# vvvm23/distributed-pytorch-cookbook

Measured on AMD Instinct MI355X. Metric: tokens/sec (node) GPT-2 training per recipe (DDP/FSDP/PP) at 1/2/4/8 MI355X, higher is better.
Workload: dtype bf16; 1 GPU; model=gpt2-small, global_batch=64, seq_len=1024, parallelism=dp1, recipe=main-ddp.py, reduce_dtype=fp32, pp_comm_dtype=fp32, step_graph=True

## Files before the change

### distributed_pytorch_cookbook_amd/ops/csrc/attention.hip

```cpp
#include "common.h"

#include <cstdlib>
#include <type_traits>

namespace dpc {

struct AttnArgs {
  const void* q; const void* k; const void* v;
  void* o;
  float* lse;
  const unsigned char* pad;
  const void* dout;
  void* dq; void* dk; void* dv;
  float* delta;
  long long ld_qkv, ld_o, ld_dqkv;
  int N, S, H;
  float scale;
  int causal;
  int hd;
  int order;
};

constexpr int KT = 64;
constexpr int QB = 128;
// ... 65 lines not shown
__device__ __forceinline__ void dma_voff(int (&v)[AT<HD>::NPW], long long ld, int wid, int lane) {
#pragma unroll
  for (int i = 0; i < AT<HD>::NPW; ++i) {
    const int prow = 8 * (wid * AT<HD>::NPW + i) + (lane >> 3);
    const int e = prow * 64 + (((lane & 7) ^ aswz(prow)) << 3);
    const int row = e / HD, chunk = (e % HD) >> 3;
    v[i] = (int)((long long)row * ld * 2 + chunk * 16);
  }
}

template <int HD>
__device__ __forceinline__ void tile_dma(const bf16_t* base, long long ld, int row0, int S, bool valid,
                                         const int (&v)[AT<HD>::NPW], bf16_t* lds, int wid) {
  const __amdgpu_buffer_rsrc_t rs = rows_rsrc(base, (unsigned)(ld * 2), row0, S, valid);
#pragma unroll
  for (int i = 0; i < AT<HD>::NPW; ++i) dma16(rs, v[i], lds + (wid * AT<HD>::NPW + i) * 512);
}

template <int HD>
__device__ __forceinline__ bf16x8 row_frag(const bf16_t* lds, int row0, int st, int lane) {
  return *reinterpret_cast<const bf16x8*>(lds + toff<HD>(row0 + (lane & 31), 2 * st + (lane >> 5)));
}

template <int HD>
__device__ __forceinline__ bf16x8 tr_frag(const bf16_t* lds, int r0, int s, int c0, int lane) {
  const int h = lane >> 5, g2 = (lane >> 4) & 1, i16 = lane & 15, q = i16 >> 2, p = i16 & 3;
  const int row = r0 + 16 * s + 4 * h + q;
  const int col = c0 + 16 * g2 + 4 * p;
  const bf16_t* a0 = lds + toff<HD>(row, col >> 3) + (col & 7);
  const bf16_t* a1 = lds + toff<HD>(row + 8, col >> 3) + (col & 7);
  short4_t lo = __builtin_amdgcn_ds_read_tr16_b64_v4i16((lds4_t)a0);
  short4_t hi = __builtin_amdgcn_ds_read_tr16_b64_v4i16((lds4_t)a1);
  typedef short short8_t __attribute__((ext_vector_type(8)));
  short8_t s8 = {lo[0], lo[1], lo[2], lo[3], hi[0], hi[1], hi[2], hi[3]};
  return __builtin_bit_cast(bf16x8, s8);
}

__device__ __forceinline__ bf16x8 acc_frag(const floatx16& x, int s) {
  uint4 u;
  u.x = pack2bf(x[8 * s + 0], x[8 * s + 1]);
  u.y = pack2bf(x[8 * s + 2], x[8 * s + 3]);
  u.z = pack2bf(x[8 * s + 4], x[8 * s + 5]);
  u.w = pack2bf(x[8 * s + 6], x[8 * s + 7]);
  return __builtin_bit_cast(bf16x8, u);
}

__device__ __forceinline__ int acc_row(int r, int lane) { return (r & 3) + 8 * (r >> 2) + 4 * (lane >> 5); }

__device__ __forceinline__ void store_pair16(bf16_t* row, int g, int hh, uint2 wa, uint2 wb) {
  const auto s0 = __builtin_amdgcn_permlane32_swap(wa.x, wb.x, false, false);
  const auto s1 = __builtin_amdgcn_permlane32_swap(wa.y, wb.y, false, false);
  *reinterpret_cast<uint4*>(row + 8 * g + 8 * hh) = make_uint4(s0[0], s1[0], s0[1], s1[1]);
}

__device__ __forceinline__ float fast_exp2(float x) { return __builtin_amdgcn_exp2f(x); }

__device__ __forceinline__ float max3f(float a, float b, float c) { return fmaxf(fmaxf(a, b), c); }

__device__ __forceinline__ unsigned long long pad_bits(const unsigned char* pad, int k0, int S, int lane) {
  if (!pad) return 0ull;
  const int k = k0 + lane;
  return __ballot(k < S && pad[k] != 0);
}

__device__ __forceinline__ bf16x8 load_row8(const bf16_t* p) {
  return *reinterpret_cast<const bf16x8*>(p);
}

#define MFMA32(a, b, c) __builtin_amdgcn_mfma_f32_32x32x16_bf16((a), (b), (c), 0, 0, 0)

__device__ __forceinline__ void scale16(floatx16& x, float a) {
#pragma unroll
  for (int i = 0; i < 16; ++i) asm volatile("v_mul_f32 %0, %0, %1" : "+v"(x[i]) : "v"(a));
}

template <int K>
__device__ __forceinline__ void zero_if_gt(floatx16& x, int r, int v) {
  asm volatile("v_cmp_lt_i32_e32 vcc, %1, %2\n\tv_cndmask_b32_e64 %0, %0, 0, vcc"
               : "+v"(x[r])
               : "n"(K), "v"(v)
               : "vcc");
}

#define DPC_RS_MUL(i) "v_mul_f32 %" #i ", %" #i ", %16\n\t"
__device__ __forceinline__ void scale16_if(floatx16& x, float a, unsigned long long up) {
  asm volatile(
      "s_cmp_eq_u64 %17, 0\n\t"
      "s_cbranch_scc1 .Ldpc_rs%=\n\t"
      "s_nop 7\n\ts_nop 7\n\t"
      DPC_RS_MUL(0) DPC_RS_MUL(1) DPC_RS_MUL(2) DPC_RS_MUL(3) DPC_RS_MUL(4) DPC_RS_MUL(5) DPC_RS_MUL(6)
      DPC_RS_MUL(7) DPC_RS_MUL(8) DPC_RS_MUL(9) DPC_RS_MUL(10) DPC_RS_MUL(11) DPC_RS_MUL(12)
      DPC_RS_MUL(13) DPC_RS_MUL(14) DPC_RS_MUL(15)
      "s_nop 7\n"
      ".Ldpc_rs%=:"
      : "+v"(x[0]), "+v"(x[1]), "+v"(x[2]), "+v"(x[3]), "+v"(x[4]), "+v"(x[5]), "+v"(x[6]), "+v"(x[7]),
        "+v"(x[8]), "+v"(x[9]), "+v"(x[10]), "+v"(x[11]), "+v"(x[12]), "+v"(x[13]), "+v"(x[14]), "+v"(x[15])
      : "v"(a), "s"(up)
      : "scc");
}
#undef DPC_RS_MUL

#define DPC_RS_MUL(i) "v_mul_f32 %" #i ", %" #i ", %17\n\t"
__device__ __forceinline__ float rescale16_if(floatx16& x, float& m, float& l, float mx, unsigned long long up) {
  float a;
  asm volatile(
      "s_cmp_eq_u64 %20, 0\n\t"
      "s_cbranch_scc1 .Ldpc_ru%=\n\t"
      "s_nop 7\n\ts_nop 7\n\t"
      "v_max_f32 %17, %16, %19\n\t"
      "v_sub_f32 %16, %16, %17\n\t"
      "v_exp_f32 %16, %16\n\t"
      "s_nop 0\n\t"
      "v_swap_b32 %16, %17\n\t"
      "v_mul_f32 %18, %18, %17\n\t"
      DPC_RS_MUL(0) DPC_RS_MUL(1) DPC_RS_MUL(2) DPC_RS_MUL(3) DPC_RS_MUL(4) DPC_RS_MUL(5) DPC_RS_MUL(6)
      DPC_RS_MUL(7) DPC_RS_MUL(8) DPC_RS_MUL(9) DPC_RS_MUL(10) DPC_RS_MUL(11) DPC_RS_MUL(12)
      DPC_RS_MUL(13) DPC_RS_MUL(14) DPC_RS_MUL(15)
      "s_nop 7\n"
      ".Ldpc_ru%=:"
      : "+v"(x[0]), "+v"(x[1]), "+v"(x[2]), "+v"(x[3]), "+v"(x[4]), "+v"(x[5]), "+v"(x[6]), "+v"(x[7]),
        "+v"(x[8]), "+v"(x[9]), "+v"(x[10]), "+v"(x[11]), "+v"(x[12]), "+v"(x[13]), "+v"(x[14]), "+v"(x[15]),
        "+v"(m), "=&v"(a), "+v"(l)
      : "v"(mx), "s"(up)
      : "scc");
  return a;
}
#undef DPC_RS_MUL

__device__ __forceinline__ void zero16(floatx16& x) {
#pragma unroll
  for (int i = 0; i < 16; ++i) x[i] = 0.f;
}

__device__ __forceinline__ int g7_local_attn(int b, int grid) {
  const int xcd = b & 7, q = grid >> 3, r = grid & 7;
  return (xcd < r ? xcd * (q + 1) : r * (q + 1) + (xcd - r) * q) + (b >> 3);
}
__device__ __forceinline__ void work_order1(int nblk, int& bh, int& i) {
  const int nbh = gridDim.x / nblk;
  i = blockIdx.x / nbh;
  bh = blockIdx.x - i * nbh;
}
__device__ __forceinline__ void xcd_work(int nblk, int& bh, int& i) {
  const int b = blockIdx.x, nwg = gridDim.x, xcd = b & 7, q = nwg >> 3, r = nwg & 7;
  const int t = (xcd < r ? xcd * (q + 1) : r * (q + 1) + (xcd - r) * q) + (b >> 3);
  bh = t / nblk;
  i = t - bh * nblk;
}

template <int HD, int OCC>
__global__ __launch_bounds__(256, OCC) void attn_fwd_kernel(AttnArgs p) {
  using A = AT<HD>;
  __shared__ __attribute__((aligned(16))) bf16_t smem[NSLOT * 2 * A::TILE];
  const int S = p.S, H = p.H;
  const int nqb = (S + QB - 1) / QB;
  int bh, bi;
  xcd_work(nqb, bh, bi);
  const int qb = nqb - 1 - bi;
  const int n = bh / H, h = bh % H;
  const int lane = threadIdx.x & 63, hh = lane >> 5;
  const int wid = __builtin_amdgcn_readfirstlane(threadIdx.x >> 6);
  const int q0 = qb * QB + wid * 32;
  const int q = q0 + (lane & 31);
  const long long tok0 = (long long)n * S;
  const bf16_t* Q = static_cast<const bf16_t*>(p.q) + h * HD;
  const bf16_t* K = static_cast<const bf16_t*>(p.k) + tok0 * p.ld_qkv + h * HD;
  const bf16_t* V = static_cast<const bf16_t*>(p.v) + tok0 * p.ld_qkv + h * HD;

  bf16x8 qf[A::NST];
#pragma unroll
  for (int st = 0; st < A::NST; ++st)
    qf[st] = q < S ? load_row8(Q + (tok0 + q) * p.ld_qkv + 16 * st + 8 * hh) : bf16x8{};
  pin_loaded(qf);
  const float c = p.scale * LOG2E;
  const int kend = p.causal ? min(S, qb * QB + QB) : S;
  const int ntiles = (kend + KT - 1) / KT;
  const int last_w = p.causal ? min(ntiles - 1, max(0, min(q0 + 31, S - 1)) / KT) : ntiles - 1;
  const unsigned char* pad = p.pad ? p.pad + (long long)n * S : nullptr;

  int dv[A::NPW];
  dma_voff<HD>(dv, p.ld_qkv, wid, lane);
  auto issue = [&](int t) {
    bf16_t* st = smem + (t % NSLOT) * 2 * A::TILE;
    const bool valid = t < ntiles;
    tile_dma<HD>(K, p.ld_qkv, t * KT, S, valid, dv, st, wid);
    tile_dma<HD>(V, p.ld_qkv, t * KT, S, valid, dv, st + A::TILE, wid);
  };
  auto qk = [&](floatx16 (&s)[2], const bf16_t* lk) {
#pragma unroll
    for (int kb = 0; kb < 2; ++kb) {
      zero16(s[kb]);
#pragma unroll
      for (int st = 0; st < A::NST; ++st)
        s[kb] = MFMA32(row_frag<HD>(lk, kb * 32, st, lane), qf[st], s[kb]);
    }
  };

  float m = -INFINITY, l = 0.f;
  floatx16 o[A::NDT];
#pragma unroll
  for (int d = 0; d < A::NDT; ++d) zero16(o[d]);

  issue(0);
  issue(1);
  issue(2);
// ... 237 lines not shown
#pragma unroll
      for (int st = 0; st < A::NST; ++st) qf[st] = row_frag<HD>(ls + (wid >> 1) * A::TILE, 32 * (wid & 1), st, lane);
      m = -INFINITY;
      l = 0.f;
#pragma unroll
      for (int d = 0; d < A::NDT; ++d) zero16(o[d]);
      qk(sn, lsn);
      return;
    }
    if (t > last_w) return;
    const bf16_t* lv = ls + A::TILE;
    const int kt0 = t * KT;
    const bool need_mask = (p.causal && kt0 + KT - 1 > q0) || (kt0 + KT > S) || pad;
    if (need_mask) {
      const int limh = (p.causal ? min(q, S - 1) : S - 1) - kt0 - 4 * hh;
      const unsigned long long pm = pad_bits(pad, kt0, S, lane) >> (4 * hh);
#pragma unroll
      for (int kb = 0; kb < 2; ++kb) {
        const unsigned pk = (unsigned)(pm >> (32 * kb));
#pragma unroll
        for (int r = 0; r < 16; ++r) {
          const int kc = kb * 32 + (r & 3) + 8 * (r >> 2);
          const bool masked = (kc > limh) || ((pk >> ((r & 3) + 8 * (r >> 2))) & 1u);
          if (masked) sc[kb][r] = -INFINITY;
        }
      }
    }
    float mq[4];
#pragma unroll
    for (int q4 = 0; q4 < 4; ++q4) {
      const floatx16& sq = sc[q4 >> 1];
      const int r0 = (q4 & 1) * 8;
      float v = max3f(sq[r0], sq[r0 + 1], sq[r0 + 2]);
      v = max3f(v, sq[r0 + 3], sq[r0 + 4]);
      v = max3f(v, sq[r0 + 5], sq[r0 + 6]);
      mq[q4] = fmaxf(v, sq[r0 + 7]);
    }
    float mx = fmaxf(max3f(mq[0], mq[1], mq[2]), mq[3]);
    {
      const auto sw = __builtin_amdgcn_permlane32_swap(__float_as_uint(mx), __float_as_uint(mx), false, false);
      mx = fmaxf(__uint_as_float(sw[0]), __uint_as_float(sw[1])) * c;
    }
    if (__ballot(mx > m + 8.f)) {
      const float mn = fmaxf(m, mx);
      const float alpha = (m == -INFINITY) ? 1.f : fast_exp2(m - mn);
      m = mn;
      l *= alpha;
#pragma unroll
      for (int d = 0; d < A::NDT; ++d) scale16(o[d], alpha);
    }
    const float nmu = (m == -INFINITY) ? 0.f : -m;
    if (t + 1 <= last_w) qk(sn, lsn);
    float lq[4] = {0.f, 0.f, 0.f, 0.f};
    bf16x8 pb[2][2];
#pragma unroll
    for (int kb = 0; kb < 2; ++kb) {
#pragma unroll
      for (int r = 0; r < 16; ++r) {
        const float ex = fast_exp2(fmaf(sc[kb][r], c, nmu));
        sc[kb][r] = ex;
        lq[r & 3] += ex;
      }
      pb[kb][0] = acc_frag(sc[kb], 0);
      pb[kb][1] = acc_frag(sc[kb], 1);
    }
    l += (lq[0] + lq[1]) + (lq[2] + lq[3]);
#pragma unroll
    for (int kb = 0; kb < 2; ++kb)
#pragma unroll
      for (int ss = 0; ss < 2; ++ss)
#pragma unroll
        for (int d = 0; d < A::NDT; ++d)
          o[d] = MFMA32(tr_frag<HD>(lv, kb * 32, ss, d * 32, lane), pb[kb][ss], o[d]);
  };
  floatx16 s0[2], s1[2];
  for (int e = 0; e < total; e += 2) {
    step(e, s0, s1);
    if (e + 1 < total) step(e + 1, s1, s0);
  }
  finish();
  vm_wait<0>();
}

template <int HD, int OCC>
__global__ __launch_bounds__(256, OCC) void attn_fwd3_kernel(AttnArgs p, int nitems) {
  using A = AT<HD>;
  __shared__ __attribute__((aligned(16))) bf16_t smem[NSLOT * 2 * A::TILE];
  const int S = p.S, H = p.H;
  const int nqb = (S + QB - 1) / QB;
  const int npr = (nqb + 1) / 2;
  const int grid = gridDim.x;
  const int local = g7_local_attn(blockIdx.x, grid);
  const int lane = threadIdx.x & 63, hh = lane >> 5;
  const int wid = __builtin_amdgcn_readfirstlane(threadIdx.x >> 6);
  auto ntiles_of = [&](int qb) {
    const int kend = p.causal ? min(S, qb * QB + QB) : S;
    return (kend + KT - 1) / KT;
  };
  auto item = [&](int k) {
    PairItem it;
    const int id = local + k * grid;
    it.bh = id / npr;
    const int pr = id - it.bh * npr;
    it.blk0 = nqb - 1 - pr;
    it.blk1 = pr;
    it.len0 = 1 + ntiles_of(it.blk0);
    it.len = it.len0 + (it.blk1 != it.blk0 ? 1 + ntiles_of(it.blk1) : 0);
    return it;
  };
  const int nmine = local < nitems ? (nitems - local + grid - 1) / grid : 0;
  if (nmine == 0) return;

  int dv[A::NPW];
  dma_voff<HD>(dv, p.ld_qkv, wid, lane);
  int is_k = 0, is_off = 0;
  PairItem is_it = item(0);
  long long is_hoff = 0;
  auto enter = [&]() {
    const int n = is_it.bh / H, h = is_it.bh - n * H;
    is_hoff = (long long)n * S * p.ld_qkv + h * HD;
  };
  enter();
  auto issue_next = [&](int e) {
    bf16_t* st = smem + (e % NSLOT) * 2 * A::TILE;
    const bool valid = is_k < nmine;
    const bool second = is_off >= is_it.len0;
    const int i = is_off - (second ? is_it.len0 : 0);
    if (i == 0 || !valid) {
      const bf16_t* base = static_cast<const bf16_t*>(p.q) + is_hoff;
      const int r0 = (second ? is_it.blk1 : is_it.blk0) * QB;
      tile_dma<HD>(base, p.ld_qkv, r0, S, valid, dv, st, wid);
      tile_dma<HD>(base, p.ld_qkv, r0 + KT, S, valid, dv, st + A::TILE, wid);
    } else {
      const bf16_t* K = static_cast<const bf16_t*>(p.k) + is_hoff;
      const bf16_t* V = static_cast<const bf16_t*>(p.v) + is_hoff;
      tile_dma<HD>(K, p.ld_qkv, (i - 1) * KT, S, true, dv, st, wid);
      tile_dma<HD>(V, p.ld_qkv, (i - 1) * KT, S, true, dv, st + A::TILE, wid);
    }
    if (valid && ++is_off == is_it.len) {
      is_off = 0;
      if (++is_k < nmine) {
        is_it = item(is_k);
        enter();
      }
    }
  };
  auto sync = [&](int e) {
    vm_wait<2 * A::NPW>();
    ring_barrier();
    issue_next(e + 3);
  };
  auto slot = [&](int e) -> const bf16_t* { return smem + (e % NSLOT) * 2 * A::TILE; };

  const float c = p.scale * LOG2E;
  bf16x8 qf[A::NST];
  float m = -INFINITY, l = 0.f;
  floatx16 o[A::NDT];
  int q0 = 0, q = 0, last_w = 0;
  int bh = 0, h = 0, n = 0;
  const unsigned char* pad = nullptr;

  auto qk = [&](floatx16 (&s)[2], const bf16_t* lk) {
#pragma unroll
    for (int kb = 0; kb < 2; ++kb) {
      zero16(s[kb]);
#pragma unroll
      for (int st = 0; st < A::NST; ++st) s[kb] = MFMA32(row_frag<HD>(lk, kb * 32, st, lane), qf[st], s[kb]);
    }
  };
  auto finish = [&]() {
    l += __shfl_xor(l, 32, 64);
    if (q < S) {
      const float inv = l > 0.f ? __builtin_amdgcn_rcpf(l) : 0.f;
      bf16_t* O = static_cast<bf16_t*>(p.o) + (long long)n * S * p.ld_o + h * HD + q * (int)p.ld_o;
#pragma unroll
      for (int d = 0; d < A::NDT; ++d)
#pragma unroll
        for (int g = 0; g < 4; g += 2) {
          uint2 wa, wb;
          wa.x = pack2bf(o[d][4 * g + 0] * inv, o[d][4 * g + 1] * inv);
          wa.y = pack2bf(o[d][4 * g + 2] * inv, o[d][4 * g + 3] * inv);
          wb.x = pack2bf(o[d][4 * g + 4] * inv, o[d][4 * g + 5] * inv);
          wb.y = pack2bf(o[d][4 * g + 6] * inv, o[d][4 * g + 7] * inv);
          store_pair16(O + d * 32, g, hh, wa, wb);
        }
      if (hh == 0) p.lse[(long long)bh * S + q] = (l > 0.f) ? (m + log2f(l)) / LOG2E : INFINITY;
    }
  };
  auto tile = [&](auto gen, int e, int t, floatx16 (&sc)[2], floatx16 (&sn)[2]) {
    constexpr bool GEN = decltype(gen)::value;
    const bf16_t* ls = slot(e);
    const bf16_t* lv = ls + A::TILE;
    const int kt0 = t * KT;
    if constexpr (GEN) {
      const bool need_mask = (p.causal && kt0 + KT - 1 > q0) || (kt0 + KT > S) || pad;
      if (need_mask) {
        const int limh = (p.causal ? min(q, S - 1) : S - 1) - kt0 - 4 * hh;
        const unsigned long long pm = pad_bits(pad, kt0, S, lane) >> (4 * hh);
#pragma unroll
        for (int kb = 0; kb < 2; ++kb) {
          const unsigned pk = (unsigned)(pm >> (32 * kb));
#pragma unroll
          for (int r = 0; r < 16; ++r) {
            const int kc = kb * 32 + (r & 3) + 8 * (r >> 2);
            const bool masked = (kc > limh) || ((pk >> ((r & 3) + 8 * (r >> 2))) & 1u);
            if (masked) sc[kb][r] = -INFINITY;
          }
        }
      }
    }
    float mq[4];
#pragma unroll
    for (int q4 = 0; q4 < 4; ++q4) {
      const floatx16& sq = sc[q4 >> 1];
      const int r0 = (q4 & 1) * 8;
      float v = max3f(sq[r0], sq[r0 + 1], sq[r0 + 2]);
      v = max3f(v, sq[r0 + 3], sq[r0 + 4]);
      v = max3f(v, sq[r0 + 5], sq[r0 + 6]);
      mq[q4] = fmaxf(v, sq[r0 + 7]);
    }
    float mx = fmaxf(max3f(mq[0], mq[1], mq[2]), mq[3]);
    {
      const auto sw = __builtin_amdgcn_permlane32_swap(__float_as_uint(mx), __float_as_uint(mx), false, false);
      mx = fmaxf(__uint_as_float(sw[0]), __uint_as_float(sw[1])) * c;
    }
    if constexpr (GEN) {
      if (__ballot(mx > m + 8.f)) {
        const float mn = fmaxf(m, mx);
        const float alpha = (m == -INFINITY) ? 1.f : fast_exp2(m - mn);
        m = mn;
        l *= alpha;
#pragma unroll
        for (int d = 0; d < A::NDT; ++d) scale16(o[d], alpha);
      }
    } else {
      const unsigned long long up = __ballot(mx > m + 8.f);
      const float alpha = rescale16_if(o[0], m, l, mx, up);
#pragma unroll
      for (int d = 1; d < A::NDT; ++d) scale16_if(o[d], alpha, up);
    }
    const float nmu = (!GEN || m != -INFINITY) ? -m : 0.f;
    if constexpr (GEN) {
      if (t + 1 <= last_w) qk(sn, slot(e + 1));
    } else {
      qk(sn, slot(e + 1));
    }
    float lq[4] = {0.f, 0.f, 0.f, 0.f};
    bf16x8 pb[2][2];
#pragma unroll
    for (int kb = 0; kb < 2; ++kb) {
#pragma unroll
      for (int r = 0; r < 16; ++r) {
        const float ex = fast_exp2(fmaf(sc[kb][r], c, nmu));
        sc[kb][r] = ex;
        lq[r & 3] += ex;
      }
      pb[kb][0] = acc_frag(sc[kb], 0);
      pb[kb][1] = acc_frag(sc[kb], 1);
    }
    l += (lq[0] + lq[1]) + (lq[2] + lq[3]);
#pragma unroll
    for (int kb = 0; kb < 2; ++kb)
#pragma unroll
      for (int ss = 0; ss < 2; ++ss)
#pragma unroll
        for (int d = 0; d < A::NDT; ++d)
          o[d] = MFMA32(tr_frag<HD>(lv, kb * 32, ss, d * 32, lane), pb[kb][ss], o[d]);
  };
  using Plain = std::integral_constant<bool, false>;
  using General = std::integral_constant<bool, true>;

  issue_next(0);
  issue_next(1);
  issue_next(2);
  floatx16 sA[2], sB[2];
  int e = 0;
  for (int k = 0; k < nmine; ++k) {
    const PairItem it = item(k);
    for (int half = 0; half < 2; ++half) {
      if (half == 1 && it.blk1 == it.blk0) break;
      const int blk = half ? it.blk1 : it.blk0;
      sync(e);
      const bf16_t* ls = slot(e);
      if (e > 0) finish();
      if (half == 0) {
        bh = it.bh;
        n = bh / H;
        h = bh - n * H;
        pad = p.pad ? p.pad + (long long)n * S : nullptr;
      }
      q0 = blk * QB + wid * 32;
      q = q0 + (lane & 31);
      const int nt = ntiles_of(blk);
      last_w = p.causal ? min(nt - 1, max(0, min(q0 + 31, S - 1)) / KT) : nt - 1;
#pragma unroll
      for (int st = 0; st < A::NST; ++st) qf[st] = row_frag<HD>(ls + (wid >> 1) * A::TILE, 32 * (wid & 1), st, lane);
      m = -INFINITY;
      l = 0.f;
#pragma unroll
      for (int d = 0; d < A::NDT; ++d) zero16(o[d]);
      qk(sA, slot(e + 1));
      ++e;
      int nf = pad ? 0 : min(last_w, S / KT);
      if (p.causal) nf = min(nf, (q0 + 1) / KT);
      int t = 0;
      for (; t + 2 <= nf; t += 2, e += 2) {
        sync(e);
        tile(Plain(), e, t, sA, sB);
        sync(e + 1);
        tile(Plain(), e + 1, t + 1, sB, sA);
      }
      if (t < nf) {
        sync(e);
        tile(Plain(), e, t, sA, sB);
#pragma unroll
        for (int kb = 0; kb < 2; ++kb) sA[kb] = sB[kb];
        ++e;
        ++t;
      }
      for (; t < nt; ++t, ++e) {
        sync(e);
        if (t <= last_w) {
          tile(General(), e, t, sA, sB);
#pragma unroll
          for (int kb = 0; kb < 2; ++kb) sA[kb] = sB[kb];
        }
      }
    }
  }
  finish();
  vm_wait<0>();
}

template <int HD, int OCC, int ABL = 0>
__global__ __launch_bounds__(256, OCC) void attn_bwd_dkdv_kernel(AttnArgs p) {
  using A = AT<HD>;
  __shared__ __attribute__((aligned(16))) bf16_t smem[NSLOT * 2 * A::TILE];
  __shared__ __attribute__((aligned(16))) float srow[NSLOT][2][KT];
  const int S = p.S, H = p.H;
  const int nkb = (S + QB - 1) / QB;
  int bh, kb;
  if (p.order == 1) work_order1(nkb, bh, kb);
  else xcd_work(nkb, bh, kb);
  const int n = bh / H, h = bh % H;
  const int lane = threadIdx.x & 63, hh = lane >> 5;
  const int wid = __builtin_amdgcn_readfirstlane(threadIdx.x >> 6);
  const int k0 = kb * QB + wid * 32;
  const int key = k0 + (lane & 31);
  const long long tok0 = (long long)n * S;
  const bf16_t* Q = static_cast<const bf16_t*>(p.q) + tok0 * p.ld_qkv + h * HD;
  const bf16_t* Kp = static_cast<const bf16_t*>(p.k) + h * HD;
  const bf16_t* Vp = static_cast<const bf16_t*>(p.v) + h * HD;
  const bf16_t* dO = static_cast<const bf16_t*>(p.dout) + tok0 * p.ld_o + h * HD;
  const float* lse = p.delta + (long long)p.N * H * S + (long long)bh * S;
  const float* delta = p.delta + (long long)bh * S;
  const bool key_ok = key < S && !(p.pad && p.pad[(long long)n * S + min(key, S - 1)]);

  bf16x8 kf[A::NST], vf[A::NST];
#pragma unroll
  for (int st = 0; st < A::NST; ++st) {
    kf[st] = bf16x8{};
    vf[st] = bf16x8{};
  }
  const float c = p.scale * LOG2E;
  floatx16 dvt[A::NDT], dkt[A::NDT];
#pragma unroll
  for (int d = 0; d < A::NDT; ++d) {
    zero16(dvt[d]);
    zero16(dkt[d]);
  }

  const int qt_begin = p.causal ? (kb * QB) / KT : 0;
  const int nqt = (S + KT - 1) / KT;
  const int count = nqt - qt_begin;

  int vq[A::NPW], vd[A::NPW];
  dma_voff<HD>(vq, p.ld_qkv, wid, lane);
  dma_voff<HD>(vd, p.ld_o, wid, lane);
  auto issue = [&](int i) {
    const int slot = i % NSLOT, qt = qt_begin + i;
    const bool valid = i < count;
    bf16_t* st = smem + slot * 2 * A::TILE;
    tile_dma<HD>(Q, p.ld_qkv, qt * KT, S, valid, vq, st, wid);
    tile_dma<HD>(dO, p.ld_o, qt * KT, S, valid, vd, st + A::TILE, wid);
    if (wid == 0) {
      dma4(rows_rsrc(lse, 4, qt * KT, S, valid), lane * 4, &srow[slot][0][0]);
      dma4(rows_rsrc(delta, 4, qt * KT, S, valid), lane * 4, &srow[slot][1][0]);
    }
  };
  auto sdp = [&](floatx16& sa, floatx16& dp, const bf16_t* lq, int r0) {
    zero16(sa);
    const float* drow = &srow[((lq - smem) / (2 * A::TILE))][1][0];
#pragma unroll
    for (int g = 0; g < 4; ++g) {
      const float4 d4 = *reinterpret_cast<const float4*>(drow + r0 + 8 * g + 4 * hh);
      dp[4 * g + 0] = d4.x;
      dp[4 * g + 1] = d4.y;
      dp[4 * g + 2] = d4.z;
      dp[4 * g + 3] = d4.w;
    }
#pragma unroll
    for (int st = 0; st < A::NST; ++st) {
      sa = MFMA32(row_frag<HD>(lq, r0, st, lane), kf[st], sa);
      dp = MFMA32(row_frag<HD>(lq + A::TILE, r0, st, lane), vf[st], dp);
    }
  };

  if (count > 0 && !(ABL & 8)) {
    if constexpr (!(ABL & 2)) {
      bf16_t* sk = smem + 2 * 2 * A::TILE;
      bf16_t* sv = smem + 3 * 2 * A::TILE;
      const bf16_t* K0 = Kp + tok0 * p.ld_qkv;
      const bf16_t* V0 = Vp + tok0 * p.ld_qkv;
      tile_dma<HD>(K0, p.ld_qkv, kb * QB, S, true, vq, sk, wid);
      tile_dma<HD>(K0, p.ld_qkv, kb * QB + KT, S, true, vq, sk + A::TILE, wid);
      tile_dma<HD>(V0, p.ld_qkv, kb * QB, S, true, vq, sv, wid);
      tile_dma<HD>(V0, p.ld_qkv, kb * QB + KT, S, true, vq, sv + A::TILE, wid);
    }
    issue(0);
    issue(1);
    if constexpr (!(ABL & 2)) {
      if (wid == 0) vm_wait<4 * A::NPW + 4>();
      else vm_wait<4 * A::NPW>();
      ring_barrier();
      const bf16_t* sk = smem + 2 * 2 * A::TILE + (wid >> 1) * A::TILE;
#pragma unroll
      for (int st = 0; st < A::NST; ++st) {
        kf[st] = row_frag<HD>(sk, 32 * (wid & 1), st, lane);
        vf[st] = row_frag<HD>(sk + 2 * A::TILE, 32 * (wid & 1), st, lane);
      }
      asm volatile("s_waitcnt lgkmcnt(0)" ::: "memory");
      __builtin_amdgcn_sched_barrier(0);
      ring_barrier();
    }
    issue(2);
    if (wid == 0) vm_wait<4 * A::NPW + 4>();
    else vm_wait<4 * A::NPW>();
    ring_barrier();
  }
  auto half = [&](int i, int hf, floatx16& sa, floatx16& dp) {
    const int slot = i % NSLOT;
    const bf16_t* lq = smem + slot * 2 * A::TILE;
    const bf16_t* ldo = lq + A::TILE;
    const int qt0 = (qt_begin + i) * KT;
    const int qs0 = qt0 + 32 * hf;
    const bool active = !(p.causal && qs0 + 31 < k0);
    if (!active) return;
    const bool diag = p.causal && qs0 < k0 + 31;
    sdp(sa, dp, lq, 32 * hf);
    sfor<4>([&](auto G) {
      constexpr int g = decltype(G)::value;
      const float4 l4 = *reinterpret_cast<const float4*>(&srow[slot][0][32 * hf + 8 * g + 4 * hh]);
      const float lv[4] = {l4.x, l4.y, l4.z, l4.w};
#pragma unroll
      for (int e = 0; e < 4; ++e) sa[4 * g + e] = fast_exp2(fmaf(sa[4 * g + e], c, -lv[e]));
    });
    if (diag) {
      const int kd = key - qs0 - 4 * hh;
      sfor<16>([&](auto R) {
        constexpr int r = decltype(R)::value;
        zero_if_gt<8 * (r >> 2) + (r & 3)>(sa, r, kd);
      });
    }
#pragma unroll
    for (int r = 0; r < 16; ++r) dp[r] = sa[r] * dp[r];
#pragma unroll
    for (int ss = 0; ss < 2; ++ss) {
      const bf16x8 pb = acc_frag(sa, ss);
      const bf16x8 db = acc_frag(dp, ss);
#pragma unroll
      for (int d = 0; d < A::NDT; ++d) {
        dvt[d] = MFMA32(tr_frag<HD>(ldo, 32 * hf, ss, d * 32, lane), pb, dvt[d]);
        dkt[d] = MFMA32(tr_frag<HD>(lq, 32 * hf, ss, d * 32, lane), db, dkt[d]);
      }
    }
  };
  floatx16 sa0, dp0, sa1, dp1;
  for (int i = 0; i < ((ABL & 1) ? 0 : count); ++i) {
    if (wid == 0) vm_wait<2 * A::NPW + 2>();
    else vm_wait<2 * A::NPW>();
    ring_barrier();
    issue(i + 3);
    half(i, 0, sa0, dp0);
    half(i, 1, sa1, dp1);
  }
  vm_wait<0>();

  if (key < S && !(ABL & 4)) {
    bf16_t* dK = static_cast<bf16_t*>(p.dk) + (tok0 + key) * p.ld_dqkv + h * HD;
    bf16_t* dV = static_cast<bf16_t*>(p.dv) + (tok0 + key) * p.ld_dqkv + h * HD;
    auto wk = [&](int d, int g) {
      uint2 w = make_uint2(0u, 0u);
      if (key_ok) {
        w.x = pack2bf(dkt[d][4 * g + 0] * p.scale, dkt[d][4 * g + 1] * p.scale);
        w.y = pack2bf(dkt[d][4 * g + 2] * p.scale, dkt[d][4 * g + 3] * p.scale);
      }
      return w;
    };
    auto wv = [&](int d, int g) {
      uint2 u = make_uint2(0u, 0u);
      if (key_ok) {
        u.x = pack2bf(dvt[d][4 * g + 0], dvt[d][4 * g + 1]);
        u.y = pack2bf(dvt[d][4 * g + 2], dvt[d][4 * g + 3]);
      }
      return u;
    };
#pragma unroll
    for (int d = 0; d < A::NDT; ++d)
#pragma unroll
      for (int g = 0; g < 4; g += 2) {
        store_pair16(dK + d * 32, g, hh, wk(d, g), wk(d, g + 1));
        store_pair16(dV + d * 32, g, hh, wv(d, g), wv(d, g + 1));
      }
  }
}

template <int HD, int OCC, int ABL = 0>
__global__ __launch_bounds__(256, OCC) void attn_bwd_dq_kernel(AttnArgs p) {
  using A = AT<HD>;
  __shared__ __attribute__((aligned(16))) bf16_t smem[NSLOT * 2 * A::TILE];
  const int S = p.S, H = p.H;
  const int nqb = (S + QB - 1) / QB;
  int bh, bi;
  if (p.order == 1) work_order1(nqb, bh, bi);
  else xcd_work(nqb, bh, bi);
  const int qb = nqb - 1 - bi;
  const int n = bh / H, h = bh % H;
  const int lane = threadIdx.x & 63, hh = lane >> 5;
  const int wid = __builtin_amdgcn_readfirstlane(threadIdx.x >> 6);
  const int q0 = qb * QB + wid * 32;
  const int q = q0 + (lane & 31);
  const long long tok0 = (long long)n * S;
  const bf16_t* Q = static_cast<const bf16_t*>(p.q) + h * HD;
  const bf16_t* K = static_cast<const bf16_t*>(p.k) + tok0 * p.ld_qkv + h * HD;
  const bf16_t* V = static_cast<const bf16_t*>(p.v) + tok0 * p.ld_qkv + h * HD;
  const bf16_t* dO = static_cast<const bf16_t*>(p.dout) + h * HD;
  const unsigned char* pad = p.pad ? p.pad + (long long)n * S : nullptr;

  bf16x8 qf[A::NST], df[A::NST];
#pragma unroll
  for (int st = 0; st < A::NST; ++st) {
    qf[st] = (q < S && !(ABL & 2)) ? load_row8(Q + (tok0 + q) * p.ld_qkv + 16 * st + 8 * hh) : bf16x8{};
    df[st] = (q < S && !(ABL & 2)) ? load_row8(dO + (tok0 + q) * p.ld_o + 16 * st + 8 * hh) : bf16x8{};
  }
  const float c = p.scale * LOG2E;
  const bf16_t* Op = static_cast<const bf16_t*>(p.o) + h * HD;
  float acc = 0.f;
  if (q < S && !(ABL & 2)) {
#pragma unroll
    for (int st = 0; st < A::NST; ++st) {
      const bf16x8 of = load_row8(Op + (tok0 + q) * p.ld_o + 16 * st + 8 * hh);
      float fo[8], fd[8];
      unpack8(__builtin_bit_cast(uint4, of), fo);
      unpack8(__builtin_bit_cast(uint4, df[st]), fd);
#pragma unroll
      for (int i = 0; i < 8; ++i) acc = fmaf(fo[i], fd[i], acc);
    }
  }
  const float dl = acc + __shfl_xor(acc, 32, 64);
  const float lse2 = q < S ? p.lse[(long long)bh * S + q] * LOG2E : INFINITY;
  if (q < S && hh == 0 && ABL == 0) {
    p.delta[(long long)bh * S + q] = -dl;
    p.delta[(long long)p.N * H * S + (long long)bh * S + q] = lse2;
  }
  pin_loaded(qf);
  pin_loaded(df);
  pin_loaded(lse2);
  pin_loaded(dl);
  floatx16 dqt[A::NDT];
#pragma unroll
  for (int d = 0; d < A::NDT; ++d) zero16(dqt[d]);

  const int kend = p.causal ? min(S, qb * QB + QB) : S;
  const int ntiles = (kend + KT - 1) / KT;

  int dv[A::NPW];
  dma_voff<HD>(dv, p.ld_qkv, wid, lane);
  auto issue = [&](int t) {
    bf16_t* st = smem + (t % NSLOT) * 2 * A::TILE;
    const bool valid = t < ntiles;
    tile_dma<HD>(K, p.ld_qkv, t * KT, S, valid, dv, st, wid);
    tile_dma<HD>(V, p.ld_qkv, t * KT, S, valid, dv, st + A::TILE, wid);
  };
  auto sdp = [&](floatx16& sa, floatx16& dp, const bf16_t* lk, int r0) {
    zero16(sa);
#pragma unroll
    for (int r = 0; r < 16; ++r) dp[r] = -dl;
#pragma unroll
    for (int st = 0; st < A::NST; ++st) {
      sa = MFMA32(row_frag<HD>(lk, r0, st, lane), qf[st], sa);
      dp = MFMA32(row_frag<HD>(lk + A::TILE, r0, st, lane), df[st], dp);
    }
  };

  if (!(ABL & 8)) {
    issue(0);
    issue(1);
    issue(2);
    vm_wait<4 * A::NPW>();
    ring_barrier();
  }
  auto half = [&](int t, int hf, floatx16& sa, floatx16& dp) {
    const bf16_t* lk = smem + (t % NSLOT) * 2 * A::TILE;
    const int kt0 = t * KT;
    const int ks0 = kt0 + 32 * hf;
    const bool active = !(p.causal && ks0 > q0 + 31);
    if (!active) return;
    const bool need_mask = (p.causal && ks0 + 31 > q0) || (ks0 + 32 > S) || pad;
    sdp(sa, dp, lk, 32 * hf);
    if (need_mask) {
      const unsigned long long pm = pad_bits(pad, kt0, S, lane);
      const int lim = (p.causal ? min(q, S - 1) : S - 1) - kt0;
#pragma unroll
      for (int r = 0; r < 16; ++r) {
        const int kl = 32 * hf + acc_row(r, lane);
        float pv = fast_exp2(fmaf(sa[r], c, -lse2));
        pv = (kl > lim || ((pm >> kl) & 1ull)) ? 0.f : pv;
        dp[r] = pv * dp[r];
      }
    } else {
#pragma unroll
      for (int r = 0; r < 16; ++r) dp[r] = fast_exp2(fmaf(sa[r], c, -lse2)) * dp[r];
    }
#pragma unroll
    for (int ss = 0; ss < 2; ++ss) {
      const bf16x8 db = acc_frag(dp, ss);
#pragma unroll
      for (int d = 0; d < A::NDT; ++d)
        dqt[d] = MFMA32(tr_frag<HD>(lk, 32 * hf, ss, d * 32, lane), db, dqt[d]);
    }
  };
  floatx16 sa0, dp0, sa1, dp1;
  for (int t = 0; t < ((ABL & 1) ? 0 : ntiles); ++t) {
    vm_wait<2 * A::NPW>();
    ring_barrier();
    issue(t + 3);
    half(t, 0, sa0, dp0);
    half(t, 1, sa1, dp1);
  }
  vm_wait<0>();

  if (q < S && !(ABL & 4)) {
    bf16_t* dQ = static_cast<bf16_t*>(p.dq) + (tok0 + q) * p.ld_dqkv + h * HD;
#pragma unroll
    for (int d = 0; d < A::NDT; ++d)
#pragma unroll
      for (int g = 0; g < 4; g += 2) {
        uint2 wa, wb;
        wa.x = pack2bf(dqt[d][4 * g + 0] * p.scale, dqt[d][4 * g + 1] * p.scale);
        wa.y = pack2bf(dqt[d][4 * g + 2] * p.scale, dqt[d][4 * g + 3] * p.scale);
        wb.x = pack2bf(dqt[d][4 * g + 4] * p.scale, dqt[d][4 * g + 5] * p.scale);
        wb.y = pack2bf(dqt[d][4 * g + 6] * p.scale, dqt[d][4 * g + 7] * p.scale);
        store_pair16(dQ + d * 32, g, hh, wa, wb);
      }
  }
}

static int launch_fwd(const AttnArgs* a, hipStream_t stream) {
  const int nqb = (a->S + QB - 1) / QB;
  const dim3 blocks((unsigned)(nqb * a->N * a->H));
  const int nitems = ((nqb + 1) / 2) * a->N * a->H;
  const dim3 pairs((unsigned)nitems);
  if (a->hd == 128) hipLaunchKernelGGL((attn_fwd_kernel<128, 1>), blocks, dim3(256), 0, stream, *a);
  else if (a->hd == 64) hipLaunchKernelGGL((attn_fwd3_kernel<64, 2>), pairs, dim3(256), 0, stream, *a, nitems);
  else if (a->S < 512) hipLaunchKernelGGL((attn_fwd2_kernel<32, 2>), pairs, dim3(256), 0, stream, *a, nitems);
  else hipLaunchKernelGGL((attn_fwd3_kernel<32, 2>), pairs, dim3(256), 0, stream, *a, nitems);
  return (int)hipGetLastError();
}

template <int HD, int OCC>
static void launch_bwd_at(const AttnArgs* a, dim3 blocks, hipStream_t stream) {
  hipLaunchKernelGGL((attn_bwd_dq_kernel<HD, OCC>), blocks, dim3(256), 0, stream, *a);
  hipLaunchKernelGGL((attn_bwd_dkdv_kernel<HD, OCC>), blocks, dim3(256), 0, stream, *a);
}
static int launch_bwd(const AttnArgs* a, hipStream_t stream) {
  const dim3 blocks((unsigned)(((a->S + QB - 1) / QB) * a->N * a->H));
  if (a->hd == 128) launch_bwd_at<128, 1>(a, blocks, stream);
  else if (a->hd == 64) launch_bwd_at<64, 2>(a, blocks, stream);
  else launch_bwd_at<32, 3>(a, blocks, stream);
  return (int)hipGetLastError();
}

}

using namespace dpc;

static bool attn_args_ok(const AttnArgs* a, bool bwd) {
  if (a->hd != 32 && a->hd != 64 && a->hd != 128) return false;
  if (a->N <= 0 || a->S <= 0 || a->H <= 0) return false;
  if (a->ld_qkv % 8 || a->ld_o % 8 || (bwd && a->ld_dqkv % 8)) return false;
  const long long ld = a->ld_qkv > a->ld_o ? a->ld_qkv : a->ld_o;
  if (((long long)a->S + 256) * ld * 2 >= 0xffffffffll) return false;
  return true;
}

DPC_API int dpc_attn_fwd(const AttnArgs* a, hipStream_t stream) {
  if (!attn_args_ok(a, false)) return (int)hipErrorInvalidValue;
  return launch_fwd(a, stream);
}

template <int ABL>
static void attn_lab_launch(const AttnArgs* a, int which, hipStream_t stream) {
  dim3 grid((unsigned)(((a->S + QB - 1) / QB) * a->N * a->H));
  if (which == 1) hipLaunchKernelGGL((attn_bwd_dkdv_kernel<64, 2, ABL>), grid, dim3(256), 0, stream, *a);
  else hipLaunchKernelGGL((attn_bwd_dq_kernel<64, 2, ABL>), grid, dim3(256), 0, stream, *a);
}
DPC_API int dpc_attn_bwd_lab(const AttnArgs* a, int which, int abl, hipStream_t stream) {
  if (!attn_args_ok(a, true) || a->hd != 64) return (int)hipErrorInvalidValue;
  if (which != 1 && which != 2) return (int)hipErrorInvalidValue;
  switch (abl) {
    case 0: attn_lab_launch<0>(a, which, stream); break;
    case 1: attn_lab_launch<1>(a, which, stream); break;
    case 2: attn_lab_launch<2>(a, which, stream); break;
    case 4: attn_lab_launch<4>(a, which, stream); break;
    case 6: attn_lab_launch<6>(a, which, stream); break;
    case 3: attn_lab_launch<3>(a, which, stream); break;
    case 5: attn_lab_launch<5>(a, which, stream); break;
    case 7: attn_lab_launch<7>(a, which, stream); break;
    case 15: attn_lab_launch<15>(a, which, stream); break;
    default: return (int)hipErrorInvalidValue;
  }
  return (int)hipGetLastError();
}


static int g_attn_order = -1;
static int attn_order() {
  if (g_attn_order < 0) g_attn_order = getenv("DPC_ATTN_ORDER") ? atoi(getenv("DPC_ATTN_ORDER")) : 1;
  return g_attn_order;
}
DPC_API void dpc_attn_set_order(int v) { g_attn_order = v; }

DPC_API int dpc_attn_bwd(const AttnArgs* a_in, hipStream_t stream) {
  AttnArgs b = *a_in;
  b.order = attn_order();
  const AttnArgs* a = &b;
  if (!attn_args_ok(a, true)) return (int)hipErrorInvalidValue;
  return launch_bwd(a, stream);
}
```

Before: 1.014 million tokens/s.

## Pin rescale registers, precompute LDS addresses, add unmasked fast path in attention backward

Several changes to the hd=64 attention kernels. The forward pair-stream kernel pins the online-softmax rescale inline asm to fixed high VGPRs (v224-v255) and caches a precomputed m+8 threshold. It also replaces pointer-based K/V fragment loads with precomputed LDS byte addresses and explicit ds_read_tr16 loads, and folds the last row max into the reduction. The dq and dkdv backward kernels gain a plain loop for fully unmasked tiles that batches both halves without causal checks, aimed at cutting per-tile branching and address arithmetic. Hardcoding register names assumes the compiler leaves those VGPRs free, which risks spills or clobbers.

```diff
diff --git a/distributed_pytorch_cookbook_amd/ops/csrc/attention.hip b/distributed_pytorch_cookbook_amd/ops/csrc/attention.hip
--- a/distributed_pytorch_cookbook_amd/ops/csrc/attention.hip
+++ b/distributed_pytorch_cookbook_amd/ops/csrc/attention.hip
@@ -171,45 +171,43 @@
                : "vcc");
 }
 
-#define DPC_RS_MUL(i) "v_mul_f32 %" #i ", %" #i ", %16\n\t"
-__device__ __forceinline__ void scale16_if(floatx16& x, float a, unsigned long long up) {
+#define DPC_RS_MUL(r) "v_mul_f32 v" #r ", v" #r ", %1\n\t"
+__device__ __forceinline__ void scale16_if_hi(floatx16& x, float a, unsigned long long up) {
   asm volatile(
-      "s_cmp_eq_u64 %17, 0\n\t"
+      "s_cmp_eq_u64 %2, 0\n\t"
       "s_cbranch_scc1 .Ldpc_rs%=\n\t"
       "s_nop 7\n\ts_nop 7\n\t"
-      DPC_RS_MUL(0) DPC_RS_MUL(1) DPC_RS_MUL(2) DPC_RS_MUL(3) DPC_RS_MUL(4) DPC_RS_MUL(5) DPC_RS_MUL(6)
-      DPC_RS_MUL(7) DPC_RS_MUL(8) DPC_RS_MUL(9) DPC_RS_MUL(10) DPC_RS_MUL(11) DPC_RS_MUL(12)
-      DPC_RS_MUL(13) DPC_RS_MUL(14) DPC_RS_MUL(15)
+      DPC_RS_MUL(240) DPC_RS_MUL(241) DPC_RS_MUL(242) DPC_RS_MUL(243) DPC_RS_MUL(244) DPC_RS_MUL(245)
+      DPC_RS_MUL(246) DPC_RS_MUL(247) DPC_RS_MUL(248) DPC_RS_MUL(249) DPC_RS_MUL(250) DPC_RS_MUL(251)
+      DPC_RS_MUL(252) DPC_RS_MUL(253) DPC_RS_MUL(254) DPC_RS_MUL(255)
       "s_nop 7\n"
       ".Ldpc_rs%=:"
-      : "+v"(x[0]), "+v"(x[1]), "+v"(x[2]), "+v"(x[3]), "+v"(x[4]), "+v"(x[5]), "+v"(x[6]), "+v"(x[7]),
-        "+v"(x[8]), "+v"(x[9]), "+v"(x[10]), "+v"(x[11]), "+v"(x[12]), "+v"(x[13]), "+v"(x[14]), "+v"(x[15])
+      : "+{v[240:255]}"(x)
       : "v"(a), "s"(up)
       : "scc");
 }
 #undef DPC_RS_MUL
 
-#define DPC_RS_MUL(i) "v_mul_f32 %" #i ", %" #i ", %17\n\t"
-__device__ __forceinline__ float rescale16_if(floatx16& x, float& m, float& l, float mx, unsigned long long up) {
+#define DPC_RS_MUL(r) "v_mul_f32 v" #r ", v" #r ", %2\n\t"
+__device__ __forceinline__ float rescale16_if(floatx16& x, float& m, float& m8, float& l, float mx, unsigned long long up) {
   float a;
   asm volatile(
-      "s_cmp_eq_u64 %20, 0\n\t"
+      "s_cmp_eq_u64 %6, 0\n\t"
       "s_cbranch_scc1 .Ldpc_ru%=\n\t"
       "s_nop 7\n\ts_nop 7\n\t"
-      "v_max_f32 %17, %16, %19\n\t"
-      "v_sub_f32 %16, %16, %17\n\t"
-      "v_exp_f32 %16, %16\n\t"
+      "v_max_f32 %2, %1, %5\n\t"
+      "v_sub_f32 %1, %1, %2\n\t"
+      "v_exp_f32 %1, %1\n\t"
       "s_nop 0\n\t"
-      "v_swap_b32 %16, %17\n\t"
-      "v_mul_f32 %18, %18, %17\n\t"
-      DPC_RS_MUL(0) DPC_RS_MUL(1) DPC_RS_MUL(2) DPC_RS_MUL(3) DPC_RS_MUL(4) DPC_RS_MUL(5) DPC_RS_MUL(6)
-      DPC_RS_MUL(7) DPC_RS_MUL(8) DPC_RS_MUL(9) DPC_RS_MUL(10) DPC_RS_MUL(11) DPC_RS_MUL(12)
-      DPC_RS_MUL(13) DPC_RS_MUL(14) DPC_RS_MUL(15)
+      "v_swap_b32 %1, %2\n\t"
+      "v_add_f32 %4, 0x41000000, %1\n\t"
+      "v_mul_f32 %3, %3, %2\n\t"
+      DPC_RS_MUL(224) DPC_RS_MUL(225) DPC_RS_MUL(226) DPC_RS_MUL(227) DPC_RS_MUL(228) DPC_RS_MUL(229)
+      DPC_RS_MUL(230) DPC_RS_MUL(231) DPC_RS_MUL(232) DPC_RS_MUL(233) DPC_RS_MUL(234) DPC_RS_MUL(235)
+      DPC_RS_MUL(236) DPC_RS_MUL(237) DPC_RS_MUL(238) DPC_RS_MUL(239)
       "s_nop 7\n"
       ".Ldpc_ru%=:"
-      : "+v"(x[0]), "+v"(x[1]), "+v"(x[2]), "+v"(x[3]), "+v"(x[4]), "+v"(x[5]), "+v"(x[6]), "+v"(x[7]),
-        "+v"(x[8]), "+v"(x[9]), "+v"(x[10]), "+v"(x[11]), "+v"(x[12]), "+v"(x[13]), "+v"(x[14]), "+v"(x[15]),
-        "+v"(m), "=&v"(a), "+v"(l)
+      : "+{v[224:239]}"(x), "+v"(m), "=&v"(a), "+v"(l), "+v"(m8)
       : "v"(mx), "s"(up)
       : "scc");
   return a;
@@ -613,9 +611,36 @@
   vm_wait<0>();
 }
 
+typedef const bf16x8 __attribute__((address_space(3)))* lds8_t;
+template <int HD>
+struct LA {
+  static constexpr int NTR = HD == 64 ? 2 : 4;
+  static constexpr int ROW32 = 32 * HD * 2;
+  static constexpr int tr_idx(int d, int j, int s) { return HD == 64 ? (d ^ j) : 2 * s + j; }
+  static constexpr int tr_off(int j, int s, int kb) { return HD == 64 ? (32 * kb + 16 * s + 8 * j) * 128 : kb * ROW32; }
+};
+template <int HD>
+__device__ __forceinline__ int tr_byte(int r0, int s, int c0, int j, int lane) {
+  const int h = lane >> 5, g2 = (lane >> 4) & 1, i16 = lane & 15, q = i16 >> 2, p = i16 & 3;
+  const int col = c0 + 16 * g2 + 4 * p;
+  return 2 * (toff<HD>(r0 + 16 * s + 4 * h + q + 8 * j, col >> 3) + (col & 7));
+}
+__device__ __forceinline__ void pin_vgpr(int& x) { asm volatile("" : "+v"(x)); }
+__device__ __forceinline__ bf16x8 lds_row16(int addr) { return *(lds8_t)(uintptr_t)(unsigned)addr; }
+__device__ __forceinline__ bf16x8 lds_tr16(int a0, int a1) {
+  short4_t lo = __builtin_amdgcn_ds_read_tr16_b64_v4i16((lds4_t)(uintptr_t)(unsigned)a0);
+  short4_t hi = __builtin_amdgcn_ds_read_tr16_b64_v4i16((lds4_t)(uintptr_t)(unsigned)a1);
+  typedef short short8_t __attribute__((ext_vector_type(8)));
+  short8_t s8 = {lo[0], lo[1], lo[2], lo[3], hi[0], hi[1], hi[2], hi[3]};
+  return __builtin_bit_cast(bf16x8, s8);
+}
+
 template <int HD, int OCC>
 __global__ __launch_bounds__(256, OCC) void attn_fwd3_kernel(AttnArgs p, int nitems) {
   using A = AT<HD>;
+  using L = LA<HD>;
+  static_assert(HD == 32 || HD == 64, "the pair-stream forward runs hd 32 / 64");
+  static_assert(OCC <= 2, "rescale16_if / scale16_if_hi name v[224:255]: the 256-register budget");
   __shared__ __attribute__((aligned(16))) bf16_t smem[NSLOT * 2 * A::TILE];
   const int S = p.S, H = p.H;
   const int nqb = (S + QB - 1) / QB;
@@ -685,18 +710,37 @@
 
   const float c = p.scale * LOG2E;
   bf16x8 qf[A::NST];
-  float m = -INFINITY, l = 0.f;
+  float m = -INFINITY, m8 = -INFINITY, l = 0.f;
   floatx16 o[A::NDT];
   int q0 = 0, q = 0, last_w = 0;
   int bh = 0, h = 0, n = 0;
   const unsigned char* pad = nullptr;
 
-  auto qk = [&](floatx16 (&s)[2], const bf16_t* lk) {
+  const int sbase = (int)(unsigned)(uintptr_t)(lds_void_t)smem;
+  int kbase[A::NST], vbase[L::NTR];
+#pragma unroll
+  for (int st = 0; st < A::NST; ++st) kbase[st] = sbase + 2 * toff<HD>(lane & 31, 2 * st + hh);
+#pragma unroll
+  for (int i = 0; i < L::NTR; ++i)
+    vbase[i] = sbase + 2 * A::TILE + (HD == 64 ? tr_byte<HD>(0, 0, 32 * i, 0, lane) : tr_byte<HD>(0, i >> 1, 0, i & 1, lane));
+#pragma unroll
+  for (int st = 0; st < A::NST; ++st) pin_vgpr(kbase[st]);
+#pragma unroll
+  for (int i = 0; i < L::NTR; ++i) pin_vgpr(vbase[i]);
+  auto slot_bytes = [&](int e) { return (e & (NSLOT - 1)) * (4 * A::TILE); };
+
+  auto qk = [&](floatx16 (&s)[2], int e) {
+    int ka[A::NST];
+#pragma unroll
+    for (int st = 0; st < A::NST; ++st) {
+      ka[st] = kbase[st] + slot_bytes(e);
+      pin_vgpr(ka[st]);
+    }
 #pragma unroll
     for (int kb = 0; kb < 2; ++kb) {
       zero16(s[kb]);
 #pragma unroll
-      for (int st = 0; st < A::NST; ++st) s[kb] = MFMA32(row_frag<HD>(lk, kb * 32, st, lane), qf[st], s[kb]);
+      for (int st = 0; st < A::NST; ++st) s[kb] = MFMA32(lds_row16(ka[st] + kb * L::ROW32), qf[st], s[kb]);
     }
   };
   auto finish = [&]() {
@@ -720,8 +764,6 @@
   };
   auto tile = [&](auto gen, int e, int t, floatx16 (&sc)[2], floatx16 (&sn)[2]) {
     constexpr bool GEN = decltype(gen)::value;
-    const bf16_t* ls = slot(e);
-    const bf16_t* lv = ls + A::TILE;
     const int kt0 = t * KT;
     if constexpr (GEN) {
       const bool need_mask = (p.causal && kt0 + KT - 1 > q0) || (kt0 + KT > S) || pad;
@@ -747,36 +789,36 @@
       const int r0 = (q4 & 1) * 8;
       float v = max3f(sq[r0], sq[r0 + 1], sq[r0 + 2]);
       v = max3f(v, sq[r0 + 3], sq[r0 + 4]);
-      v = max3f(v, sq[r0 + 5], sq[r0 + 6]);
-      mq[q4] = fmaxf(v, sq[r0 + 7]);
-    }
-    float mx = fmaxf(max3f(mq[0], mq[1], mq[2]), mq[3]);
+      mq[q4] = max3f(v, sq[r0 + 5], sq[r0 + 6]);
+    }
+    float mx = max3f(max3f(mq[0], mq[1], mq[2]), mq[3], max3f(sc[0][7], sc[0][15], sc[1][7]));
+    mx = fmaxf(mx, sc[1][15]);
     {
       const auto sw = __builtin_amdgcn_permlane32_swap(__float_as_uint(mx), __float_as_uint(mx), false, false);
       mx = fmaxf(__uint_as_float(sw[0]), __uint_as_float(sw[1])) * c;
     }
     if constexpr (GEN) {
-      if (__ballot(mx > m + 8.f)) {
+      if (__ballot(mx > m8)) {
         const float mn = fmaxf(m, mx);
         const float alpha = (m == -INFINITY) ? 1.f : fast_exp2(m - mn);
         m = mn;
+        m8 = mn + 8.f;
         l *= alpha;
 #pragma unroll
         for (int d = 0; d < A::NDT; ++d) scale16(o[d], alpha);
       }
     } else {
-      const unsigned long long up = __ballot(mx > m + 8.f);
-      const float alpha = rescale16_if(o[0], m, l, mx, up);
-#pragma unroll
-      for (int d = 1; d < A::NDT; ++d) scale16_if(o[d], alpha, up);
+      const unsigned long long up = __ballot(mx > m8);
+      const float alpha = rescale16_if(o[0], m, m8, l, mx, up);
+      if constexpr (A::NDT == 2) scale16_if_hi(o[1], alpha, up);
     }
     const float nmu = (!GEN || m != -INFINITY) ? -m : 0.f;
     if constexpr (GEN) {
-      if (t + 1 <= last_w) qk(sn, slot(e + 1));
+      if (t + 1 <= last_w) qk(sn, e + 1);
     } else {
-      qk(sn, slot(e + 1));
-    }
-    float lq[4] = {0.f, 0.f, 0.f, 0.f};
+      qk(sn, e + 1);
+    }
+    float lq[4];
     bf16x8 pb[2][2];
 #pragma unroll
     for (int kb = 0; kb < 2; ++kb) {
@@ -784,19 +826,27 @@
       for (int r = 0; r < 16; ++r) {
         const float ex = fast_exp2(fmaf(sc[kb][r], c, nmu));
         sc[kb][r] = ex;
-        lq[r & 3] += ex;
+        if (kb == 0 && r < 4) lq[r] = ex;
+        else lq[r & 3] += ex;
       }
       pb[kb][0] = acc_frag(sc[kb], 0);
       pb[kb][1] = acc_frag(sc[kb], 1);
     }
     l += (lq[0] + lq[1]) + (lq[2] + lq[3]);
+    int va[L::NTR];
+#pragma unroll
+    for (int i = 0; i < L::NTR; ++i) {
+      va[i] = vbase[i] + slot_bytes(e);
+      pin_vgpr(va[i]);
+    }
 #pragma unroll
     for (int kb = 0; kb < 2; ++kb)
 #pragma unroll
       for (int ss = 0; ss < 2; ++ss)
 #pragma unroll
         for (int d = 0; d < A::NDT; ++d)
-          o[d] = MFMA32(tr_frag<HD>(lv, kb * 32, ss, d * 32, lane), pb[kb][ss], o[d]);
+          o[d] = MFMA32(lds_tr16(va[L::tr_idx(d, 0, ss)] + L::tr_off(0, ss, kb), va[L::tr_idx(d, 1, ss)] + L::tr_off(1, ss, kb)),
+                        pb[kb][ss], o[d]);
   };
   using Plain = std::integral_constant<bool, false>;
   using General = std::integral_constant<bool, true>;
@@ -827,10 +877,11 @@
 #pragma unroll
       for (int st = 0; st < A::NST; ++st) qf[st] = row_frag<HD>(ls + (wid >> 1) * A::TILE, 32 * (wid & 1), st, lane);
       m = -INFINITY;
+      m8 = -INFINITY;
       l = 0.f;
 #pragma unroll
       for (int d = 0; d < A::NDT; ++d) zero16(o[d]);
-      qk(sA, slot(e + 1));
+      qk(sA, e + 1);
       ++e;
       int nf = pad ? 0 : min(last_w, S / KT);
       if (p.causal) nf = min(nf, (q0 + 1) / KT);
@@ -863,7 +914,7 @@
   vm_wait<0>();
 }
 
-template <int HD, int OCC, int ABL = 0>
+template <int HD, int OCC, int ABL = 0, int PLAIN = 1>
 __global__ __launch_bounds__(256, OCC) void attn_bwd_dkdv_kernel(AttnArgs p) {
   using A = AT<HD>;
   __shared__ __attribute__((aligned(16))) bf16_t smem[NSLOT * 2 * A::TILE];
@@ -969,23 +1020,38 @@
     else vm_wait<4 * A::NPW>();
     ring_barrier();
   }
+  auto pexp = [&](int slot, int hf, floatx16& sa) {
+    sfor<4>([&](auto G) {
+      constexpr int g = decltype(G)::value;
+      const float4 l4 = *reinterpret_cast<const float4*>(&srow[slot][0][32 * hf + 8 * g + 4 * hh]);
+      const float lv[4] = {l4.x, l4.y, l4.z, l4.w};
+#pragma unroll
+      for (int e = 0; e < 4; ++e) sa[4 * g + e] = fast_exp2(fmaf(sa[4 * g + e], c, -lv[e]));
+    });
+  };
+  auto accum = [&](const bf16_t* lq, int hf, const floatx16& sa, const floatx16& dp) {
+    const bf16_t* ldo = lq + A::TILE;
+#pragma unroll
+    for (int ss = 0; ss < 2; ++ss) {
+      const bf16x8 pb = acc_frag(sa, ss);
+      const bf16x8 db = acc_frag(dp, ss);
+#pragma unroll
+      for (int d = 0; d < A::NDT; ++d) {
+        dvt[d] = MFMA32(tr_frag<HD>(ldo, 32 * hf, ss, d * 32, lane), pb, dvt[d]);
+        dkt[d] = MFMA32(tr_frag<HD>(lq, 32 * hf, ss, d * 32, lane), db, dkt[d]);
+      }
+    }
+  };
   auto half = [&](int i, int hf, floatx16& sa, floatx16& dp) {
     const int slot = i % NSLOT;
     const bf16_t* lq = smem + slot * 2 * A::TILE;
-    const bf16_t* ldo = lq + A::TILE;
     const int qt0 = (qt_begin + i) * KT;
     const int qs0 = qt0 + 32 * hf;
     const bool active = !(p.causal && qs0 + 31 < k0);
     if (!active) return;
     const bool diag = p.causal && qs0 < k0 + 31;
     sdp(sa, dp, lq, 32 * hf);
-    sfor<4>([&](auto G) {
-      constexpr int g = decltype(G)::value;
-      const float4 l4 = *reinterpret_cast<const float4*>(&srow[slot][0][32 * hf + 8 * g + 4 * hh]);
-      const float lv[4] = {l4.x, l4.y, l4.z, l4.w};
-#pragma unroll
-      for (int e = 0; e < 4; ++e) sa[4 * g + e] = fast_exp2(fmaf(sa[4 * g + e], c, -lv[e]));
-    });
+    pexp(slot, hf, sa);
     if (diag) {
       const int kd = key - qs0 - 4 * hh;
       sfor<16>([&](auto R) {
@@ -995,23 +1061,46 @@
     }
 #pragma unroll
     for (int r = 0; r < 16; ++r) dp[r] = sa[r] * dp[r];
-#pragma unroll
-    for (int ss = 0; ss < 2; ++ss) {
-      const bf16x8 pb = acc_frag(sa, ss);
-      const bf16x8 db = acc_frag(dp, ss);
-#pragma unroll
-      for (int d = 0; d < A::NDT; ++d) {
-        dvt[d] = MFMA32(tr_frag<HD>(ldo, 32 * hf, ss, d * 32, lane), pb, dvt[d]);
-        dkt[d] = MFMA32(tr_frag<HD>(lq, 32 * hf, ss, d * 32, lane), db, dkt[d]);
-      }
-    }
+    accum(lq, hf, sa, dp);
   };
   floatx16 sa0, dp0, sa1, dp1;
-  for (int i = 0; i < ((ABL & 1) ? 0 : count); ++i) {
+  auto plain = [&](int i) {
+    const int slot = i % NSLOT;
+    const bf16_t* lq = smem + slot * 2 * A::TILE;
+    sdp(sa0, dp0, lq, 0);
+    sdp(sa1, dp1, lq, 32);
+    pexp(slot, 0, sa0);
+#pragma unroll
+    for (int r = 0; r < 16; ++r) dp0[r] = sa0[r] * dp0[r];
+    pexp(slot, 1, sa1);
+#pragma unroll
+    for (int r = 0; r < 16; ++r) dp1[r] = sa1[r] * dp1[r];
+    accum(lq, 0, sa0, dp0);
+    accum(lq, 1, sa1, dp1);
+  };
+  auto sync = [&](int i) {
     if (wid == 0) vm_wait<2 * A::NPW + 2>();
     else vm_wait<2 * A::NPW>();
     ring_barrier();
     issue(i + 3);
+  };
+  const int n_run = (ABL & 1) ? 0 : count;
+  const int i_lo = min(n_run, p.pad ? n_run : (p.causal ? (k0 + 31 - qt_begin * KT + KT - 1) / KT : 0));
+  const int i_hi = min(n_run, max(i_lo, S / KT - qt_begin));
+  int i = 0;
+  if constexpr (PLAIN != 0) {
+    for (; i < i_lo; ++i) {
+      sync(i);
+      half(i, 0, sa0, dp0);
+      half(i, 1, sa1, dp1);
+    }
+    for (; i < i_hi; ++i) {
+      sync(i);
+      plain(i);
+    }
+  }
+  for (; i < n_run; ++i) {
+    sync(i);
     half(i, 0, sa0, dp0);
     half(i, 1, sa1, dp1);
   }
@@ -1046,7 +1135,7 @@
   }
 }
 
-template <int HD, int OCC, int ABL = 0>
+template <int HD, int OCC, int ABL = 0, int PLAIN = 1>
 __global__ __launch_bounds__(256, OCC) void attn_bwd_dq_kernel(AttnArgs p) {
   using A = AT<HD>;
   __shared__ __attribute__((aligned(16))) bf16_t smem[NSLOT * 2 * A::TILE];
@@ -1131,6 +1220,15 @@
     vm_wait<4 * A::NPW>();
     ring_barrier();
   }
+  auto accum = [&](const bf16_t* lk, int hf, const floatx16& dp) {
+#pragma unroll
+    for (int ss = 0; ss < 2; ++ss) {
+      const bf16x8 db = acc_frag(dp, ss);
+#pragma unroll
+      for (int d = 0; d < A::NDT; ++d)
+        dqt[d] = MFMA32(tr_frag<HD>(lk, 32 * hf, ss, d * 32, lane), db, dqt[d]);
+    }
+  };
   auto half = [&](int t, int hf, floatx16& sa, floatx16& dp) {
     const bf16_t* lk = smem + (t % NSLOT) * 2 * A::TILE;
     const int kt0 = t * KT;
@@ -1153,19 +1251,37 @@
 #pragma unroll
       for (int r = 0; r < 16; ++r) dp[r] = fast_exp2(fmaf(sa[r], c, -lse2)) * dp[r];
     }
-#pragma unroll
-    for (int ss = 0; ss < 2; ++ss) {
-      const bf16x8 db = acc_frag(dp, ss);
-#pragma unroll
-      for (int d = 0; d < A::NDT; ++d)
-        dqt[d] = MFMA32(tr_frag<HD>(lk, 32 * hf, ss, d * 32, lane), db, dqt[d]);
-    }
+    accum(lk, hf, dp);
   };
   floatx16 sa0, dp0, sa1, dp1;
-  for (int t = 0; t < ((ABL & 1) ? 0 : ntiles); ++t) {
+  auto plain = [&](int t) {
+    const bf16_t* lk = smem + (t % NSLOT) * 2 * A::TILE;
+    sdp(sa0, dp0, lk, 0);
+    sdp(sa1, dp1, lk, 32);
+#pragma unroll
+    for (int r = 0; r < 16; ++r) dp0[r] = fast_exp2(fmaf(sa0[r], c, -lse2)) * dp0[r];
+#pragma unroll
+    for (int r = 0; r < 16; ++r) dp1[r] = fast_exp2(fmaf(sa1[r], c, -lse2)) * dp1[r];
+    accum(lk, 0, dp0);
+    accum(lk, 1, dp1);
+  };
+  auto sync = [&](int t) {
     vm_wait<2 * A::NPW>();
     ring_barrier();
     issue(t + 3);
+  };
+  const int n_run = (ABL & 1) ? 0 : ntiles;
+  int t = 0;
+  if constexpr (PLAIN != 0) {
+    int nf = pad ? 0 : min(n_run, S / KT);
+    if (p.causal) nf = min(nf, (q0 + 1) / KT);
+    for (; t < nf; ++t) {
+      sync(t);
+      plain(t);
+    }
+  }
+  for (; t < n_run; ++t) {
+    sync(t);
     half(t, 0, sa0, dp0);
     half(t, 1, sa1, dp1);
   }
@@ -1201,8 +1317,9 @@
 
 template <int HD, int OCC>
 static void launch_bwd_at(const AttnArgs* a, dim3 blocks, hipStream_t stream) {
-  hipLaunchKernelGGL((attn_bwd_dq_kernel<HD, OCC>), blocks, dim3(256), 0, stream, *a);
-  hipLaunchKernelGGL((attn_bwd_dkdv_kernel<HD, OCC>), blocks, dim3(256), 0, stream, *a);
+  constexpr int PLAIN = HD == 64;
+  hipLaunchKernelGGL((attn_bwd_dq_kernel<HD, OCC, 0, PLAIN>), blocks, dim3(256), 0, stream, *a);
+  hipLaunchKernelGGL((attn_bwd_dkdv_kernel<HD, OCC, 0, PLAIN>), blocks, dim3(256), 0, stream, *a);
 }
 static int launch_bwd(const AttnArgs* a, hipStream_t stream) {
   const dim3 blocks((unsigned)(((a->S + QB - 1) / QB) * a->N * a->H));
```

After: 1.016 million tokens/s, median of 6. No clear change (+0.3%).
